# mcveanlab/Corticall

Measured on AMD Instinct MI355X. Metric: k-mers traversed/sec (whole node) + contigs/sec, k=47 3-color LdBG, higher is better.
Workload: dtype u64

## Files before the change

### corticall_amd/csrc/walk.cpp

```cpp
#include <algorithm>
#include <chrono>
#include <numeric>
#include <thread>

#include "lscoop.h"
#include "runs.h"
#include "runstep.h"
#include "shard.h"
#include "strand.h"

namespace ldbg {

#define LDBG_STREAM_BLOCK 64
#define LDBG_STREAM_GRID 65536

LDBG_DEV void walk_finish(const WalkArgs& a, StrandState& st) {
    strand_finish(a, st);
    const bool good = !st.branch_null && st.status == ST_OK;
    a.strand_n[st.s] = good ? st.gV : 0u;
    a.strand_c[st.s] = good ? st.pw.n : 0u;
}

template <int W>
LDBG_DEV bool strand_step(const WalkArgs& a, StrandState& st, LinkStoreDev& ls, const StepPre& pre, RunState& rs) {
// ... 474 lines not shown
}
template <int W>
LDBG_KERNEL void k_contigs(ContigArgs a) {
    const int k = a.g.k;
    const int64_t wave = global_tid() >> 6, lane = global_tid() & 63, nwaves = (global_nthreads() + 63) >> 6;
    for (int64_t i = wave; i < a.n; i += nwaves) {
        if (a.walk_len[i] == 0) continue;
        const int64_t L = a.contig_off[i + 1] - a.contig_off[i];
        const int64_t ro = a.strand_off[2 * i], nr = a.strand_off[2 * i + 1] - ro;
        const int64_t fo = a.strand_off[2 * i + 1];
        const int64_t nrev = nr > 0 ? nr - 1 : 0;
        char* o = a.out + a.contig_off[i];
        if (a.quirk[2 * i] | a.quirk[2 * i + 1]) {
            for (int64_t p = lane; p < L; p += 64) {
                const int64_t v = p < k ? 0 : p - k + 1;
                const Kmer<W> km = walk_vertex_kmer<W>(a, i, v, ro, nr, fo);
                o[p] = "ACGT"[kmer_base<W>(km, k, p < k ? (int)p : k - 1)];
            }
            continue;
        }
        Kmer<W> sk;
#pragma unroll
        for (int w = 0; w < W; w++) sk.w[w] = a.seeds[i * W + w];
        for (int64_t p = lane; p < L; p += 64) {
            unsigned b;
            if (p < nrev) b = path_base(a.dense[ro + (nr - 1 - p)]);
            else if (p < nrev + k) b = kmer_base<W>(sk, k, (int)(p - nrev));
            else b = path_base(a.dense[fo + (p - nrev - k + 1)]);
            o[p] = "ACGT"[b];
        }
    }
}

struct ContigRleArgs {
    GraphView g;
    RunIndexView runs;
    int64_t n;
    const uint64_t* seeds;
    const uint64_t* pool; const uint32_t* block_table; int max_blocks;
    const uint32_t* strand_c; const uint32_t* strand_n;
    const int64_t* walk_len; const int64_t* contig_off;
    char* out;
};
LDBG_DEV uint64_t rle_stored(const ContigRleArgs& a, int64_t s, uint32_t j) {
    return a.pool[(uint64_t)a.block_table[s * a.max_blocks + j / LDBG_PATH_BLOCK] * LDBG_PATH_BLOCK + (j & (LDBG_PATH_BLOCK - 1))];
}
template <int W>
LDBG_KERNEL void k_contigs_rle(ContigRleArgs a) {
    const int k = a.g.k;
    const int64_t wave = global_tid() / wave_size(), nwaves = (global_nthreads() + wave_size() - 1) / wave_size();
    const uint32_t lane = (uint32_t)wave_lane(), WS = (uint32_t)wave_size();
    for (int64_t i = wave; i < a.n; i += nwaves) {
        if (a.walk_len[i] == 0) continue;
        char* o = a.out + a.contig_off[i];
        const int64_t nr = a.strand_n[2 * i], nrev = nr > 0 ? nr - 1 : 0;
        Kmer<W> sk;
#pragma unroll
        for (int w = 0; w < W; w++) sk.w[w] = a.seeds[i * W + w];
        for (uint32_t p = lane; p < (uint32_t)k; p += WS) o[nrev + p] = "ACGT"[kmer_base<W>(sk, k, (int)p)];
        for (int dir = 0; dir < 2; dir++) {
            const int64_t s = 2 * i + dir;
            const bool fwd = dir == 1;
            const uint32_t nc = a.strand_c[s];
            auto place = [&](uint32_t v) -> int64_t { return fwd ? nrev + k - 1 + (int64_t)v : nrev - (int64_t)v; };
            uint32_t base_v = 0;
            uint64_t carry = 0;
            for (uint32_t j0 = 0; j0 < nc; j0 += WS) {
                const uint32_t j = j0 + lane;
                const uint64_t* blk = a.pool + (uint64_t)a.block_table[s * a.max_blocks + j0 / LDBG_PATH_BLOCK] * LDBG_PATH_BLOCK;
                const uint64_t e = j < nc ? LDBG_GLOBAL(const uint64_t, blk)[j & (LDBG_PATH_BLOCK - 1)] : 0ull;
                const uint64_t up = wave_shfl_u64(e, (int)lane - 1);
                const uint64_t prev = (j & (LDBG_PATH_BLOCK - 1)) == 0u ? 0ull : (lane == 0u ? carry : up);
                carry = wave_shfl_u64(e, (int)WS - 1);
                const uint32_t cnt = j < nc ? pd_expanded(prev, e) : 0u;
                const uint32_t incl = wave_incl_scan_u32(cnt);
                const uint32_t at = base_v + incl - cnt;
                const bool head = cnt > 0u && pd_is_head(e);
                if (cnt == 1u && !head && at >= 1u) o[place(at)] = "ACGT"[path_base(e)];
                const bool is_run = head && LDBG_PD_KIND(e) == LDBG_PD_RUN;
                unsigned long long hb = wave_ballot(is_run);
                const uint32_t GS = WS == 64u ? 16u : WS, g = lane / GS, sub = lane % GS;
                const uint8_t* ub = LDBG_GLOBAL(const uint8_t, a.runs.ubase);
                while (hb) {
                    uint32_t myL = 0;
                    bool gv = false;
                    for (uint32_t q = 0; q < WS / GS; q++) {
                        if (!hb) break;
                        const int L = __builtin_ctzll(hb);
                        hb &= hb - 1;
                        if (g == q) { myL = (uint32_t)L; gv = true; }
                    }
                    const uint64_t he = wave_shfl_u64(e, (int)myL);
                    const uint32_t hat = wave_shfl_u32(at, (int)myL), len_of = wave_shfl_u32(cnt, (int)myL);
                    const uint32_t len = gv ? len_of : 0u;
                    const uint64_t next_e = wave_shfl_u64(e, (int)myL + 1);
                    const uint64_t payload = !gv ? 0ull : (myL + 1u < WS ? next_e : rle_stored(a, s, j0 + myL + 1u));
                    const bool asc = (he >> 36) & 1ull, inv = (he >> 37) & 1ull;
                    const uint32_t first = (uint32_t)payload;
                    const unsigned shift = (fwd != inv) ? 2u : 0u, comp = inv ? 3u : 0u;
                    auto ascii = [&](unsigned bb) -> unsigned { return (0x54474341u >> (8u * (((bb >> shift) & 3u) ^ comp))) & 0xFFu; };
                    auto ascii4 = [&](uint32_t bb4) -> uint32_t {
                        const uint32_t f = ((bb4 >> shift) & 0x03030303u) ^ (comp * 0x01010101u);
#ifndef LDBG_HOSTSIM
                        return __builtin_amdgcn_perm(0u, 0x54474341u, f);
#else
                        uint32_t v = 0;
                        for (int bI = 0; bI < 4; bI++) v |= ((0x54474341u >> (8u * ((f >> (8 * bI)) & 3u))) & 0xFFu) << (8 * bI);
                        return v;
#endif
                    };
                    const uint8_t* in_lo = asc ? ub + first : ub + first - (len ? len - 1u : 0u);
                    char* out_lo = LDBG_GLOBAL(char, o) + (fwd ? place(hat) : place(hat + (len ? len - 1u : 0u)));
                    const bool same = asc == fwd;
                    const uint32_t nd = len / 8u;
                    uint32_t max_nd = wave_bcast_u32(nd, 0);
                    for (uint32_t q = 1; q < WS / GS; q++) { const uint32_t o2 = wave_bcast_u32(nd, (int)(q * GS)); max_nd = o2 > max_nd ? o2 : max_nd; }
                    for (uint32_t base = 0; base < max_nd; base += 4u * GS) {
                        uint64_t w[4];
#pragma unroll
                        for (int q = 0; q < 4; q++) {
                            const uint32_t ci = base + (uint32_t)q * GS + sub;
                            w[q] = 0;
                            if (ci < nd) __builtin_memcpy(&w[q], in_lo + (same ? 8u * ci : len - 8u - 8u * ci), 8);
                        }
#pragma unroll
                        for (int q = 0; q < 4; q++) {
                            const uint32_t ci = base + (uint32_t)q * GS + sub;
                            uint64_t v = (uint64_t)ascii4((uint32_t)w[q]) | ((uint64_t)ascii4((uint32_t)(w[q] >> 32)) << 32);
                            if (!same) v = __builtin_bswap64(v);
                            if (ci < nd) __builtin_memcpy(out_lo + 8u * ci, &v, 8);
                        }
                    }
                    for (uint32_t t = 8u * nd + sub; t < len; t += GS) {
                        const unsigned bb = in_lo[same ? t : len - 1u - t];
                        out_lo[t] = (char)ascii(bb);
                    }
                }
                hb = wave_ballot(head && !is_run);
                while (hb) {
                    const int L = __builtin_ctzll(hb);
                    hb &= hb - 1;
                    const uint32_t hat = wave_bcast_u32(at, L), len = wave_bcast_u32(cnt, L);
                    const uint64_t payload = (uint32_t)L + 1u < WS ? wave_bcast_u64(e, L + 1) : rle_stored(a, s, j0 + (uint32_t)L + 1);
                    wave_fence();
                    const uint32_t first = (uint32_t)payload, period = (uint32_t)(payload >> 32);
                    const uint32_t nch = (len + 7u) / 8u;
                    for (uint32_t c = lane; c < nch; c += WS) {
                        const uint32_t t0 = 8u * c, m = len - t0 < 8u ? len - t0 : 8u;
                        uint32_t r = t0 % period;
                        uint64_t v = 0;
#pragma unroll
                        for (uint32_t b = 0; b < 8u; b++) {
                            if (b < m) {
                                const uint64_t ch = (uint8_t)LDBG_GLOBAL(const char, o)[place(first + period + r)];
                                v |= ch << (8u * (fwd ? b : m - 1u - b));
                            }
                            r++;
                            if (r == period) r = 0;
                        }
                        char* lo = LDBG_GLOBAL(char, o) + (fwd ? place(hat + t0) : place(hat + t0 + m - 1u));
                        if (m == 8u) __builtin_memcpy(lo, &v, 8);
                        else for (uint32_t b = 0; b < m; b++) lo[b] = (char)(v >> (8u * b));
                    }
                }
                base_v += wave_bcast_u32(incl, (int)WS - 1);
            }
        }
    }
}

template <int W>
LDBG_KERNEL void k_walk_vertices(GraphView g, const uint64_t* dense, int64_t ro, int64_t nr, int64_t fo, int64_t nf,
                                 const uint64_t* term_r, const uint64_t* term_f, int64_t len, uint64_t* words, int64_t* rec,
                                 int32_t* copy, int32_t* index) {
    const int64_t nrev = nr > 0 ? nr - 1 : 0;
    for (int64_t p = global_tid(); p < len; p += global_nthreads()) {
        uint64_t e;
        int idx_label;
        const uint64_t* term;
        if (p < nrev) { e = dense[ro + (nr - 1 - p)]; idx_label = -1; term = term_r; }
        else if (p == nrev) { e = nr > 0 ? dense[ro] : dense[fo]; idx_label = 0; term = nullptr; }
        else { e = dense[fo + (p - nrev)]; idx_label = 1; term = term_f; }
        int64_t ri = path_idx(e);
        Kmer<W> km;
        if (ri >= 0) {
            km = graph_key<W>(g, ri);
            if (path_flip(e)) km = kmer_revcomp<W>(km, g.k);
        } else {
            for (int w = 0; w < W; w++) km.w[w] = term ? term[w] : 0;
        }
        for (int w = 0; w < W; w++) words[p * W + w] = km.w[w];
        rec[p] = ri;
        copy[p] = path_copy(e);
        index[p] = idx_label;
    }
}

struct RoiHitArgs {
    const uint32_t* roi_of;
    int64_t n;
    const uint64_t* dense; const int64_t* strand_off; const int64_t* walk_len;
// ... 630 lines not shown
        if (!us.empty())
            fprintf(stderr, "[ldbg] %zu strands of %u iterations: us/iter p0/p10/p50/p90/p100 = %.2f %.2f %.2f %.2f %.2f\n", us.size(), max_it,
                    us[0], us[us.size() / 10], us[us.size() / 2], us[us.size() * 9 / 10], us.back());
    }
    double tot_ms = 0; for (int64_t i = 0; i < ns; i++) tot_ms += (tt[2 * i + 1] - tt[2 * i]) / 1e5;
    fprintf(stderr, "[ldbg] sum of strand durations %.1f s over %lld strands; %llu wavefront loop iterations in %d wavefronts\n", tot_ms / 1e3, (long long)ns,
            ctr[14], grid);
    rt::dfree(a.st_times);
}

bool Engine::walk_finish(WalkRun& r, int64_t* traversed) {
    rt::stream_t s = stream_;
    const WalkArgs& a = r.a;
    WalkChunk& out = r.out;
    const int64_t n = r.n, ns = r.ns;
    HostLaps laps;

    if (!h_small_) h_small_ = (unsigned long long*)rt::hmalloc_pinned(64 * 8);
    unsigned long long* const ctr = h_small_;
    if (runs_ && !a.img_on) {
        r.d_retry = (uint32_t*)rt::tmalloc((size_t)ns * 4);
        LDBG_LAUNCH(k_retry_list, grid_for(ns, 256, 1024), 256, s, (const uint32_t*)r.d_status, ns, r.d_retry, r.d_ctr + 28);
        rt::d2h(ctr, r.d_ctr, 256, s);
        rt::stream_sync(s);
        if (r.timed) { r.walk_ms += rt::Event::elapsed_ms(r.ev0, r.ev1); r.timed = false; }
        const int64_t n_again = (int64_t)ctr[28];
        if (n_again > 0) {
            rt::dmemset(r.d_ctr, 0, 8, s);
            WalkArgs b = a;
            b.e.runs = RunIndexView{nullptr, nullptr, nullptr};
            b.retry = r.d_retry;
            b.n_strands = n_again;
            retried_strands_ += n_again;
            launch_k_walk(r, b, s);
        }
    }

    int64_t* d_walk_len = (int64_t*)rt::tmalloc((size_t)n * 8);
    uint8_t* d_seed_ok = (uint8_t*)rt::tmalloc((size_t)n);
    uint32_t* d_contig_len = (uint32_t*)rt::tmalloc((size_t)n * 4);
    int64_t* d_strand_off = (int64_t*)rt::tmalloc((size_t)(ns + 1) * 8);
    int64_t* d_contig_off = (int64_t*)rt::tmalloc((size_t)(n + 1) * 8);
    unsigned long long* d_scan = (unsigned long long*)rt::tmalloc((size_t)(2 * OFF_SCAN_OWNERS + 2) * 8);
    auto free_results = [&] {
        rt::tfree(d_walk_len); rt::tfree(d_seed_ok); rt::tfree(d_contig_len); rt::tfree(d_strand_off); rt::tfree(d_contig_off); rt::tfree(d_scan);
        d_walk_len = nullptr; d_seed_ok = nullptr; d_contig_len = nullptr; d_strand_off = nullptr; d_contig_off = nullptr; d_scan = nullptr;
    };
    AsmArgs aa;
    aa.e = view; aa.n = n; aa.op_and = cfg.combination_operator == LDBG_OP_AND; aa.k = r.k;
    aa.seeds = a.seeds; aa.pool = a.pool; aa.block_table = a.block_table; aa.max_blocks = r.max_blocks;
    aa.strand_n = r.d_strand_n; aa.status = r.d_status; aa.iters = r.d_iters; aa.quirk = r.d_quirk;
    aa.walk_len = d_walk_len; aa.seed_ok = d_seed_ok; aa.contig_len = d_contig_len; aa.flags = r.d_ctr + 24;
    LDBG_LAUNCH(k_walk_lengths, grid_for(n, 256, 2048), 256, s, aa);
    int64_t* d_totals = (int64_t*)(d_scan + 2 * OFF_SCAN_OWNERS);
    launch_offsets(r.d_strand_n, ns, d_strand_off, d_scan, d_totals, s);
    launch_offsets(d_contig_len, n, d_contig_off, d_scan + OFF_SCAN_OWNERS, d_totals + 1, s);
    rt::d2h(ctr, r.d_ctr, 256, s);
    rt::d2h(ctr + 32, d_totals, 16, s);
    rt::stream_sync(s);
    if (r.timed) { r.walk_ms += rt::Event::elapsed_ms(r.ev0, r.ev1); r.timed = false; }
    {
        static const char* const kind_names[8] = {"walk_steps_run", "walk_run_vertices", "walk_steps_lean", "walk_steps_general", "walk_link_adds", "walk_choices",
                                                  "walk_wave_iterations", "walk_wave_general"};
        for (int q = 0; q < 8; q++) profile_add(kind_names[q], (double)ctr[8 + q]);
        profile_add("walk_busiest_general", (double)(ctr[16] >> 32));
        profile_add("walk_busiest_iterations", (double)(ctr[16] & 0xFFFFFFFFull));
// ... 14 lines not shown

    if (pool_full) {
        r.discard(); free_results();
        return false;
    }
    if (any_error) {
        for (int64_t i = 0; i < ns; i++) {
            const uint32_t st = out.status[i];
            if (st != ST_NULLPTR && st != ST_LINKSTORE_FULL && st != ST_COPY_OVERFLOW) continue;
            r.discard(); free_results();
            if (st == ST_NULLPTR)
                throw StatusError(LDBG_ERR_NULLPOINTER, "getNextVertices: record missing while recruitment colours are set (seed " + std::to_string(r.first + i / 2) + ")");
            if (st == ST_LINKSTORE_FULL) throw StatusError(LDBG_ERR_CAPACITY, "LINKSTORE_FULL");
            throw StatusError(LDBG_ERR_UNSUPPORTED, "a vertex was visited more than 32767 times in one walk");
        }
    }
    *traversed += (int64_t)ctr[27];
    out.total_entries = (int64_t)ctr[32];
    out.total_bytes = (int64_t)ctr[33];
    out.host_ready = false;

    const bool lazy = !any_quirk && r.first == 0 && n == batch_n && !getenv("LDBG_EAGER_PATHS");
    out.d_contigs = result_alloc((size_t)out.total_bytes, &out.contigs_cap);
    out.d_strand_off = d_strand_off; d_strand_off = nullptr;
    out.d_contig_off = d_contig_off;
    out.d_walk_len = d_walk_len;
    out.d_strand_c = r.d_strand_c; r.d_strand_c = nullptr;
    out.max_blocks = r.max_blocks;
    out.runs = a.e.runs;
    out.dense_pending = true;
    laps.lap("result buffers");
    rt::Event c0, c1;
    c0.record(s);
    if (lazy) {
        ContigRleArgs ra;
        ra.g = graph->view; ra.runs = a.e.runs; ra.n = n; ra.seeds = a.seeds;
        ra.pool = (const uint64_t*)d_pool_; ra.block_table = (const uint32_t*)d_block_table_; ra.max_blocks = r.max_blocks;
        ra.strand_c = (const uint32_t*)out.d_strand_c; ra.strand_n = r.d_strand_n; ra.walk_len = d_walk_len; ra.contig_off = d_contig_off;
        ra.out = (char*)out.d_contigs;
        int rb = LDBG_STREAM_BLOCK, rcap = LDBG_STREAM_GRID;
#ifndef LDBG_HOSTSIM
        if (const char* ev = getenv("LDBG_RLE_BLOCK")) rb = atoi(ev) >= 256 ? 256 : (atoi(ev) >= 128 ? 128 : 64);
        if (const char* ev = getenv("LDBG_RLE_GRID")) rcap = std::max(1, atoi(ev));
#endif
        LDBG_LAUNCH_W(r.W, k_contigs_rle, grid_for(n * 64, rb, rcap), rb, s, ra);
    } else {
        ensure_dense(out);
        ContigArgs ca;
        ca.g = graph->view; ca.n = n; ca.seeds = a.seeds; ca.dense = (const uint64_t*)out.d_path; ca.strand_off = (const int64_t*)out.d_strand_off;
        ca.walk_len = d_walk_len; ca.contig_off = d_contig_off; ca.quirk = r.d_quirk; ca.term = (const uint64_t*)out.d_term;
        ca.out = (char*)out.d_contigs;
        LDBG_LAUNCH_W(r.W, k_contigs, grid_for(n * 64), 256, s, ca);
    }
    c1.record(s);
    rt::stream_sync(s);
    profile_add("contig", rt::Event::elapsed_ms(c0, c1));
    laps.lap("paths + contigs");
    r.free_tmp();
    d_walk_len = nullptr; d_contig_off = nullptr;
    free_results();
    laps.lap("frees");
    return true;
}


void Engine::sharded_walk_begin(ShardImage& img, const char* seeds, int64_t n, const int32_t* d_seed_slot, rt::stream_t round_stream) {
    if (cfg.stopping_rule != LDBG_STOP_CONTIG || cfg.connect_all_neighbors || cfg.n_secondary > 0)
        throw StatusError(LDBG_ERR_UNSUPPORTED, "walks over a sharded table run ContigStopper without connectAllNeighbors / secondary colours");
    if (&img.graph() != graph) throw StatusError(LDBG_ERR_ARG, "the engine was not created on this image's graph");
    enter();
    sharded_abort();
    clear_batch();
    seeds_to_device(seeds, n, false);
    batch_n = n;
    sharded_run_ = new WalkRun;
    sharded_img_ = &img;
    sharded_stream_ = round_stream ? round_stream : stream_;
    try {
        walk_prepare(0, n, *sharded_run_, &img, d_seed_slot);
        rt::stream_sync(stream_);
    } catch (...) { sharded_abort(); throw; }
}
void Engine::sharded_abort() {
    if (sharded_run_) {
        quiesce();
        sharded_run_->discard();
        delete sharded_run_;
        sharded_run_ = nullptr;
    }
    sharded_img_ = nullptr;
}
// ... 138 lines not shown
```

Before: 187.3 billion.

## Restructure RLE contig emission into a per-wave run table with a flattened chunk copy

The RLE contig kernel now preloads the first two wave-groups of path entries for both strands and hoists the per-contig metadata loads. It builds a shared-memory table of run descriptors and then copies all run chunks in one flat, software-pipelined pass across lanes, instead of handling runs four at a time in 16-lane groups. The goal is to remove lane imbalance and serialized per-run loops in contig materialization. In exchange it adds shared-memory use, binary searches over the table, extra fences, a fallback path for long strands, and the block size is now fixed at 64 threads per block.

```diff
diff --git a/corticall_amd/csrc/walk.cpp b/corticall_amd/csrc/walk.cpp
--- a/corticall_amd/csrc/walk.cpp
+++ b/corticall_amd/csrc/walk.cpp
@@ -540,131 +540,260 @@
     const int64_t* walk_len; const int64_t* contig_off;
     char* out;
 };
-LDBG_DEV uint64_t rle_stored(const ContigRleArgs& a, int64_t s, uint32_t j) {
-    return a.pool[(uint64_t)a.block_table[s * a.max_blocks + j / LDBG_PATH_BLOCK] * LDBG_PATH_BLOCK + (j & (LDBG_PATH_BLOCK - 1))];
+struct alignas(16) RleRun {
+    uint32_t c0;
+    uint32_t in_lo;
+    uint32_t out_lo;
+    uint32_t lenf;
+};
+#define LDBG_RLE_TABLE 64u
+#define LDBG_RLE_HELD 2
+LDBG_DEV uint32_t ascii4(uint32_t bb4, unsigned shift, unsigned comp) {
+    const uint32_t f = ((bb4 >> shift) & 0x03030303u) ^ (comp * 0x01010101u);
+#ifndef LDBG_HOSTSIM
+    return __builtin_amdgcn_perm(0u, 0x54474341u, f);
+#else
+    uint32_t v = 0;
+    for (int bI = 0; bI < 4; bI++) v |= ((0x54474341u >> (8u * ((f >> (8 * bI)) & 3u))) & 0xFFu) << (8 * bI);
+    return v;
+#endif
 }
 template <int W>
-LDBG_KERNEL void k_contigs_rle(ContigRleArgs a) {
-    const int k = a.g.k;
+LDBG_DEV void contigs_rle_wave(const int k, const int64_t n, const int max_blocks, const uint64_t* __restrict__ seeds, const uint64_t* __restrict__ pool,
+                               const uint32_t* __restrict__ block_table, const uint32_t* __restrict__ strand_c, const uint32_t* __restrict__ strand_n,
+                               const int64_t* __restrict__ walk_len, const int64_t* __restrict__ contig_off, const uint8_t* __restrict__ ubase,
+                               char* __restrict__ out, RleRun* tab) {
     const int64_t wave = global_tid() / wave_size(), nwaves = (global_nthreads() + wave_size() - 1) / wave_size();
     const uint32_t lane = (uint32_t)wave_lane(), WS = (uint32_t)wave_size();
-    for (int64_t i = wave; i < a.n; i += nwaves) {
-        if (a.walk_len[i] == 0) continue;
-        char* o = a.out + a.contig_off[i];
-        const int64_t nr = a.strand_n[2 * i], nrev = nr > 0 ? nr - 1 : 0;
+    const uint8_t* ub = LDBG_GLOBAL(const uint8_t, ubase);
+    for (int64_t i = wave; i < n; i += nwaves) {
+        const int64_t wl = walk_len[i], co = contig_off[i];
+        const uint32_t nr = strand_n[2 * i], nc0 = strand_c[2 * i], nc1 = strand_c[2 * i + 1];
+        const uint32_t bt0 = block_table[(2 * i) * max_blocks], bt1 = block_table[(2 * i + 1) * max_blocks];
         Kmer<W> sk;
 #pragma unroll
-        for (int w = 0; w < W; w++) sk.w[w] = a.seeds[i * W + w];
+        for (int w = 0; w < W; w++) sk.w[w] = seeds[i * W + w];
+        if (wl == 0) continue;
+        char* o = out + co;
+        const uint32_t nrev = nr > 0u ? nr - 1u : 0u;
+        auto place = [&](bool fwd, uint32_t v) -> uint32_t { return fwd ? nrev + (uint32_t)k - 1u + v : nrev - v; };
+        uint64_t e[2][LDBG_RLE_HELD], ex[2];
+#pragma unroll
+        for (int d = 0; d < 2; d++) {
+            const uint32_t nc = d ? nc1 : nc0;
+            const uint64_t* blk = pool + (uint64_t)(d ? bt1 : bt0) * LDBG_PATH_BLOCK;
+#pragma unroll
+            for (int g = 0; g < LDBG_RLE_HELD; g++) {
+                const uint32_t j = (uint32_t)g * WS + lane;
+                e[d][g] = j < nc ? LDBG_GLOBAL(const uint64_t, blk)[j] : 0ull;
+            }
+            ex[d] = LDBG_RLE_HELD * WS < nc ? LDBG_GLOBAL(const uint64_t, blk)[LDBG_RLE_HELD * WS] : 0ull;
+        }
         for (uint32_t p = lane; p < (uint32_t)k; p += WS) o[nrev + p] = "ACGT"[kmer_base<W>(sk, k, (int)p)];
-        for (int dir = 0; dir < 2; dir++) {
-            const int64_t s = 2 * i + dir;
-            const bool fwd = dir == 1;
-            const uint32_t nc = a.strand_c[s];
-            auto place = [&](uint32_t v) -> int64_t { return fwd ? nrev + k - 1 + (int64_t)v : nrev - (int64_t)v; };
-            uint32_t base_v = 0;
-            uint64_t carry = 0;
-            for (uint32_t j0 = 0; j0 < nc; j0 += WS) {
+
+        struct Group { uint32_t at, cnt; bool is_run, is_rep; uint64_t payload; };
+        auto scan_group = [&](bool fwd, uint32_t j0, uint32_t nc, uint64_t ge, uint64_t after, uint64_t& carry, uint32_t& base_v) -> Group {
+            Group r;
+            const uint32_t j = j0 + lane;
+            const uint64_t up = wave_shfl_u64(ge, (int)lane - 1), dn = wave_shfl_u64(ge, (int)lane + 1);
+            const uint64_t prev = (j & (LDBG_PATH_BLOCK - 1)) == 0u ? 0ull : (lane == 0u ? carry : up);
+            carry = wave_shfl_u64(ge, (int)WS - 1);
+            r.payload = lane + 1u < WS ? dn : after;
+            r.cnt = j < nc ? pd_expanded(prev, ge) : 0u;
+            const uint32_t incl = wave_incl_scan_u32(r.cnt);
+            r.at = base_v + incl - r.cnt;
+            const bool head = r.cnt > 0u && pd_is_head(ge);
+            if (r.cnt == 1u && !head && r.at >= 1u) o[place(fwd, r.at)] = "ACGT"[path_base(ge)];
+            r.is_run = head && LDBG_PD_KIND(ge) == LDBG_PD_RUN;
+            r.is_rep = head && !r.is_run;
+            base_v += wave_bcast_u32(incl, (int)WS - 1);
+            return r;
+        };
+        auto table_add = [&](bool fwd, uint64_t ge, const Group& gr, uint32_t& R, uint32_t& C) {
+            const unsigned long long hb = wave_ballot(gr.is_run);
+            const uint32_t len = gr.is_run ? gr.cnt : 0u, nch = (len + 7u) / 8u;
+            const uint32_t incl = wave_incl_scan_u32(nch);
+            if (gr.is_run) {
+                const bool asc = (ge >> 36) & 1ull, inv = (ge >> 37) & 1ull;
+                const uint32_t first = (uint32_t)gr.payload, span = len ? len - 1u : 0u;
+                RleRun t;
+                t.c0 = C + incl - nch;
+                t.in_lo = asc ? first : first - span;
+                t.out_lo = fwd ? place(fwd, gr.at) : place(fwd, gr.at + span);
+                t.lenf = len | ((asc == fwd) ? 1u << 20 : 0u) | ((fwd != inv) ? 1u << 21 : 0u) | (inv ? 1u << 22 : 0u);
+                tab[R + (uint32_t)wave_count_below(hb)] = t;
+            }
+            R += (uint32_t)__builtin_popcountll(hb);
+            C += wave_bcast_u32(incl, (int)WS - 1);
+        };
+        auto copy_pass = [&](const uint32_t R, const uint32_t C) {
+            if (R == 0u || C == 0u) return;
+            uint32_t r = 0, nxt = 0;
+            RleRun cur = tab[0];
+            auto load1 = [&](uint32_t c, uint64_t& w, uint32_t& oo, uint32_t& mf) {
+                w = 0; oo = 0; mf = 0;
+                if (c >= C) return;
+                if (c >= nxt) {
+                    uint32_t lo = r, hi = R;
+                    while (hi - lo > 1u) { const uint32_t mid = (lo + hi) >> 1; if (tab[mid].c0 <= c) lo = mid; else hi = mid; }
+                    r = lo; cur = tab[r]; nxt = r + 1u < R ? tab[r + 1u].c0 : 0xFFFFFFFFu;
+                }
+                const uint32_t len = cur.lenf & 0xFFFFFu, t0 = 8u * (c - cur.c0), m = len - t0 < 8u ? len - t0 : 8u;
+                const bool same = (cur.lenf >> 20) & 1u;
+                oo = cur.out_lo + t0; mf = m | ((cur.lenf >> 20) << 4);
+                const uint8_t* in = ub + cur.in_lo;
+                if (len >= 8u) {
+                    const uint32_t x = same ? (t0 < len - 8u ? t0 : len - 8u) : (len - 8u > t0 ? len - 8u - t0 : 0u);
+                    __builtin_memcpy(&w, in + x, 8);
+                } else {
+#pragma unroll
+                    for (uint32_t b = 0; b < 7u; b++)
+                        if (b < len) w |= (uint64_t)in[b] << (8u * (same ? b + 8u - len : b));
+                }
+            };
+            auto store1 = [&](uint64_t w, uint32_t oo, uint32_t mf) {
+                const uint32_t m = mf & 15u;
+                if (!m) return;
+                const unsigned shift = (mf >> 5) & 1u ? 2u : 0u, comp = (mf >> 6) & 1u ? 3u : 0u;
+                uint64_t v = (uint64_t)ascii4((uint32_t)w, shift, comp) | ((uint64_t)ascii4((uint32_t)(w >> 32), shift, comp) << 32);
+                if (!((mf >> 4) & 1u)) v = __builtin_bswap64(v);
+                v >>= 8u * (8u - m);
+                char* p = LDBG_GLOBAL(char, o) + oo;
+                if (m == 8u) __builtin_memcpy(p, &v, 8);
+                else {
+#pragma unroll
+                    for (uint32_t b = 0; b < 7u; b++)
+                        if (b < m) p[b] = (char)(v >> (8u * b));
+                }
+            };
+            const uint32_t NB = (C + 4u * WS - 1u) / (4u * WS);
+            uint64_t wa[4], wb[4];
+            uint32_t oa[4], ob[4], ma[4], mb[4];
+#pragma unroll
+            for (uint32_t q = 0; q < 4u; q++) load1(q * WS + lane, wa[q], oa[q], ma[q]);
+            for (uint32_t b = 0; b < NB; b++) {
+#pragma unroll
+                for (uint32_t q = 0; q < 4u; q++) load1((4u * (b + 1u) + q) * WS + lane, wb[q], ob[q], mb[q]);
+#pragma unroll
+                for (uint32_t q = 0; q < 4u; q++) store1(wa[q], oa[q], ma[q]);
+#pragma unroll
+                for (uint32_t q = 0; q < 4u; q++) { wa[q] = wb[q]; oa[q] = ob[q]; ma[q] = mb[q]; }
+            }
+        };
+        auto repeat_tail = [&](bool fwd, uint32_t hat, uint32_t len, uint64_t payload) {
+            wave_fence();
+            const uint32_t first = (uint32_t)payload, period = (uint32_t)(payload >> 32);
+            const uint32_t nch = (len + 7u) / 8u;
+            for (uint32_t c = lane; c < nch; c += WS) {
+                const uint32_t t0 = 8u * c, m = len - t0 < 8u ? len - t0 : 8u;
+                uint32_t r = t0 % period;
+                uint64_t v = 0;
+#pragma unroll
+                for (uint32_t b = 0; b < 8u; b++) {
+                    if (b < m) {
+                        const uint64_t ch = (uint8_t)LDBG_GLOBAL(const char, o)[place(fwd, first + period + r)];
+                        v |= ch << (8u * (fwd ? b : m - 1u - b));
+                    }
+                    r++;
+                    if (r == period) r = 0;
+                }
+                char* lo = LDBG_GLOBAL(char, o) + (fwd ? place(fwd, hat + t0) : place(fwd, hat + t0 + m - 1u));
+                if (m == 8u) __builtin_memcpy(lo, &v, 8);
+                else for (uint32_t b = 0; b < m; b++) lo[b] = (char)(v >> (8u * b));
+            }
+        };
+        auto repeat_of = [&](bool fwd, const Group& gr) {
+            const unsigned long long hb = wave_ballot(gr.is_rep);
+            if (!hb) return;
+            const int L = __builtin_ctzll(hb);
+            repeat_tail(fwd, wave_bcast_u32(gr.at, L), wave_bcast_u32(gr.cnt, L), wave_bcast_u64(gr.payload, L));
+        };
+
+        Group gr[2][LDBG_RLE_HELD];
+        uint64_t carry[2] = {0ull, 0ull};
+        uint32_t base_v[2] = {0u, 0u}, heads = 0;
+#pragma unroll
+        for (int d = 0; d < 2; d++) {
+            const uint32_t nc = d ? nc1 : nc0;
+#pragma unroll
+            for (int g = 0; g < LDBG_RLE_HELD; g++) {
+                const uint64_t after = g + 1 < LDBG_RLE_HELD ? wave_bcast_u64(e[d][g + 1 < LDBG_RLE_HELD ? g + 1 : g], 0) : ex[d];
+                gr[d][g] = scan_group(d == 1, (uint32_t)g * WS, nc, e[d][g], after, carry[d], base_v[d]);
+                heads += (uint32_t)__builtin_popcountll(wave_ballot(gr[d][g].is_run));
+            }
+        }
+        const bool joint = heads <= LDBG_RLE_TABLE;
+#pragma nounroll
+        for (int pass = 0; pass < (joint ? 1 : 2); pass++) {
+            uint32_t R = 0, C = 0;
+#pragma unroll
+            for (int d = 0; d < 2; d++) {
+                if (!joint && d != pass) continue;
+#pragma unroll
+                for (int g = 0; g < LDBG_RLE_HELD; g++) table_add(d == 1, e[d][g], gr[d][g], R, C);
+            }
+            wave_fence();
+            copy_pass(R, C);
+            wave_fence();
+        }
+#pragma nounroll
+        for (int d = 0; d < 2; d++) {
+            Group last = gr[0][0];
+#pragma unroll
+            for (int g = 0; g < LDBG_RLE_HELD; g++) {
+                const Group& x = d ? gr[1][g] : gr[0][g];
+                if (g == 0) last = x;
+                else { const bool any = wave_ballot(x.is_rep) != 0ull; if (any) last = x; }
+            }
+            repeat_of(d == 1, last);
+        }
+
+#pragma nounroll
+        for (int d = 0; d < 2; d++) {
+            const uint32_t nc = d ? nc1 : nc0;
+            if (nc <= LDBG_RLE_HELD * WS) continue;
+            const bool fwd = d == 1;
+            const uint32_t* btp = block_table + (2 * i + d) * max_blocks;
+            uint32_t bcur = d ? bt1 : bt0, bnext = nc > LDBG_PATH_BLOCK ? btp[1] : 0u;
+            uint64_t cy = d ? carry[1] : carry[0];
+            uint32_t bv = d ? base_v[1] : base_v[0];
+            auto entries = [&](uint32_t j0) -> uint64_t {
                 const uint32_t j = j0 + lane;
-                const uint64_t* blk = a.pool + (uint64_t)a.block_table[s * a.max_blocks + j0 / LDBG_PATH_BLOCK] * LDBG_PATH_BLOCK;
-                const uint64_t e = j < nc ? LDBG_GLOBAL(const uint64_t, blk)[j & (LDBG_PATH_BLOCK - 1)] : 0ull;
-                const uint64_t up = wave_shfl_u64(e, (int)lane - 1);
-                const uint64_t prev = (j & (LDBG_PATH_BLOCK - 1)) == 0u ? 0ull : (lane == 0u ? carry : up);
-                carry = wave_shfl_u64(e, (int)WS - 1);
-                const uint32_t cnt = j < nc ? pd_expanded(prev, e) : 0u;
-                const uint32_t incl = wave_incl_scan_u32(cnt);
-                const uint32_t at = base_v + incl - cnt;
-                const bool head = cnt > 0u && pd_is_head(e);
-                if (cnt == 1u && !head && at >= 1u) o[place(at)] = "ACGT"[path_base(e)];
-                const bool is_run = head && LDBG_PD_KIND(e) == LDBG_PD_RUN;
-                unsigned long long hb = wave_ballot(is_run);
-                const uint32_t GS = WS == 64u ? 16u : WS, g = lane / GS, sub = lane % GS;
-                const uint8_t* ub = LDBG_GLOBAL(const uint8_t, a.runs.ubase);
-                while (hb) {
-                    uint32_t myL = 0;
-                    bool gv = false;
-                    for (uint32_t q = 0; q < WS / GS; q++) {
-                        if (!hb) break;
-                        const int L = __builtin_ctzll(hb);
-                        hb &= hb - 1;
-                        if (g == q) { myL = (uint32_t)L; gv = true; }
+                return j < nc ? LDBG_GLOBAL(const uint64_t, pool + (uint64_t)bcur * LDBG_PATH_BLOCK)[j & (LDBG_PATH_BLOCK - 1)] : 0ull;
+            };
+            uint64_t ec = entries(LDBG_RLE_HELD * WS);
+            for (uint32_t j0 = LDBG_RLE_HELD * WS; j0 < nc; j0 += WS) {
+                const uint32_t jn = j0 + WS;
+                uint64_t en = 0;
+                if (jn < nc) {
+                    if ((jn & (LDBG_PATH_BLOCK - 1)) == 0u) {
+                        const uint32_t bi = jn / LDBG_PATH_BLOCK + 1u;
+                        bcur = bnext;
+                        bnext = (uint64_t)bi * LDBG_PATH_BLOCK < nc ? btp[bi] : 0u;
                     }
-                    const uint64_t he = wave_shfl_u64(e, (int)myL);
-                    const uint32_t hat = wave_shfl_u32(at, (int)myL), len_of = wave_shfl_u32(cnt, (int)myL);
-                    const uint32_t len = gv ? len_of : 0u;
-                    const uint64_t next_e = wave_shfl_u64(e, (int)myL + 1);
-                    const uint64_t payload = !gv ? 0ull : (myL + 1u < WS ? next_e : rle_stored(a, s, j0 + myL + 1u));
-                    const bool asc = (he >> 36) & 1ull, inv = (he >> 37) & 1ull;
-                    const uint32_t first = (uint32_t)payload;
-                    const unsigned shift = (fwd != inv) ? 2u : 0u, comp = inv ? 3u : 0u;
-                    auto ascii = [&](unsigned bb) -> unsigned { return (0x54474341u >> (8u * (((bb >> shift) & 3u) ^ comp))) & 0xFFu; };
-                    auto ascii4 = [&](uint32_t bb4) -> uint32_t {
-                        const uint32_t f = ((bb4 >> shift) & 0x03030303u) ^ (comp * 0x01010101u);
+                    en = entries(jn);
+                }
+                const Group x = scan_group(fwd, j0, nc, ec, wave_bcast_u64(en, 0), cy, bv);
+                uint32_t R = 0, C = 0;
+                table_add(fwd, ec, x, R, C);
+                wave_fence();
+                copy_pass(R, C);
+                wave_fence();
+                repeat_of(fwd, x);
+                ec = en;
+            }
+        }
+    }
+}
+template <int W>
+LDBG_WAVE_KERNEL void k_contigs_rle(ContigRleArgs a) {
 #ifndef LDBG_HOSTSIM
-                        return __builtin_amdgcn_perm(0u, 0x54474341u, f);
+    __shared__ RleRun tab[LDBG_RLE_TABLE];
 #else
-                        uint32_t v = 0;
-                        for (int bI = 0; bI < 4; bI++) v |= ((0x54474341u >> (8u * ((f >> (8 * bI)) & 3u))) & 0xFFu) << (8 * bI);
-                        return v;
-#endif
-                    };
-                    const uint8_t* in_lo = asc ? ub + first : ub + first - (len ? len - 1u : 0u);
-                    char* out_lo = LDBG_GLOBAL(char, o) + (fwd ? place(hat) : place(hat + (len ? len - 1u : 0u)));
-                    const bool same = asc == fwd;
-                    const uint32_t nd = len / 8u;
-                    uint32_t max_nd = wave_bcast_u32(nd, 0);
-                    for (uint32_t q = 1; q < WS / GS; q++) { const uint32_t o2 = wave_bcast_u32(nd, (int)(q * GS)); max_nd = o2 > max_nd ? o2 : max_nd; }
-                    for (uint32_t base = 0; base < max_nd; base += 4u * GS) {
-                        uint64_t w[4];
-#pragma unroll
-                        for (int q = 0; q < 4; q++) {
-                            const uint32_t ci = base + (uint32_t)q * GS + sub;
-                            w[q] = 0;
-                            if (ci < nd) __builtin_memcpy(&w[q], in_lo + (same ? 8u * ci : len - 8u - 8u * ci), 8);
-                        }
-#pragma unroll
-                        for (int q = 0; q < 4; q++) {
-                            const uint32_t ci = base + (uint32_t)q * GS + sub;
-                            uint64_t v = (uint64_t)ascii4((uint32_t)w[q]) | ((uint64_t)ascii4((uint32_t)(w[q] >> 32)) << 32);
-                            if (!same) v = __builtin_bswap64(v);
-                            if (ci < nd) __builtin_memcpy(out_lo + 8u * ci, &v, 8);
-                        }
-                    }
-                    for (uint32_t t = 8u * nd + sub; t < len; t += GS) {
-                        const unsigned bb = in_lo[same ? t : len - 1u - t];
-                        out_lo[t] = (char)ascii(bb);
-                    }
-                }
-                hb = wave_ballot(head && !is_run);
-                while (hb) {
-                    const int L = __builtin_ctzll(hb);
-                    hb &= hb - 1;
-                    const uint32_t hat = wave_bcast_u32(at, L), len = wave_bcast_u32(cnt, L);
-                    const uint64_t payload = (uint32_t)L + 1u < WS ? wave_bcast_u64(e, L + 1) : rle_stored(a, s, j0 + (uint32_t)L + 1);
-                    wave_fence();
-                    const uint32_t first = (uint32_t)payload, period = (uint32_t)(payload >> 32);
-                    const uint32_t nch = (len + 7u) / 8u;
-                    for (uint32_t c = lane; c < nch; c += WS) {
-                        const uint32_t t0 = 8u * c, m = len - t0 < 8u ? len - t0 : 8u;
-                        uint32_t r = t0 % period;
-                        uint64_t v = 0;
-#pragma unroll
-                        for (uint32_t b = 0; b < 8u; b++) {
-                            if (b < m) {
-                                const uint64_t ch = (uint8_t)LDBG_GLOBAL(const char, o)[place(first + period + r)];
-                                v |= ch << (8u * (fwd ? b : m - 1u - b));
-                            }
-                            r++;
-                            if (r == period) r = 0;
-                        }
-                        char* lo = LDBG_GLOBAL(char, o) + (fwd ? place(hat + t0) : place(hat + t0 + m - 1u));
-                        if (m == 8u) __builtin_memcpy(lo, &v, 8);
-                        else for (uint32_t b = 0; b < m; b++) lo[b] = (char)(v >> (8u * b));
-                    }
-                }
-                base_v += wave_bcast_u32(incl, (int)WS - 1);
-            }
-        }
-    }
+    static thread_local RleRun tab[LDBG_RLE_TABLE];
+#endif
+    contigs_rle_wave<W>(a.g.k, a.n, a.max_blocks, a.seeds, a.pool, a.block_table, a.strand_c, a.strand_n, a.walk_len, a.contig_off,
+                        a.runs.ubase, a.out, tab);
 }
 
 template <int W>
@@ -1447,12 +1576,11 @@
         ra.pool = (const uint64_t*)d_pool_; ra.block_table = (const uint32_t*)d_block_table_; ra.max_blocks = r.max_blocks;
         ra.strand_c = (const uint32_t*)out.d_strand_c; ra.strand_n = r.d_strand_n; ra.walk_len = d_walk_len; ra.contig_off = d_contig_off;
         ra.out = (char*)out.d_contigs;
-        int rb = LDBG_STREAM_BLOCK, rcap = LDBG_STREAM_GRID;
+        int rcap = LDBG_STREAM_GRID;
 #ifndef LDBG_HOSTSIM
-        if (const char* ev = getenv("LDBG_RLE_BLOCK")) rb = atoi(ev) >= 256 ? 256 : (atoi(ev) >= 128 ? 128 : 64);
         if (const char* ev = getenv("LDBG_RLE_GRID")) rcap = std::max(1, atoi(ev));
 #endif
-        LDBG_LAUNCH_W(r.W, k_contigs_rle, grid_for(n * 64, rb, rcap), rb, s, ra);
+        LDBG_LAUNCH_W(r.W, k_contigs_rle, grid_for(n * 64, LDBG_STREAM_BLOCK, rcap), LDBG_STREAM_BLOCK, s, ra);
     } else {
         ensure_dense(out);
         ContigArgs ca;
```

After: 190.0 billion, median of 6. +1.4%, better.

## Split RLE contig emission into per-strand scan, work-queue copy, and repeat kernels

Applied to the files above, without the earlier changes.

The per-contig RLE kernel now assigns one wave per strand instead of per contig. Instead of copying run payloads inline, it emits fixed-size copy work items (runs cut into pieces) and repeat items into global queues through atomic counters. Separate kernels then drain those queues: a grouped copy kernel for runs and a wave-per-item kernel for periodic repeats. This is meant to remove the load imbalance from long runs serialised within one wave. The cost is extra launches, temporary buffers sized from counters, and atomics, and the repeat kernel relies on earlier output being complete before it runs.

```diff
diff --git a/corticall_amd/csrc/walk.cpp b/corticall_amd/csrc/walk.cpp
--- a/corticall_amd/csrc/walk.cpp
+++ b/corticall_amd/csrc/walk.cpp
@@ -530,6 +530,16 @@
     }
 }
 
+#define LDBG_CONTIG_CUT 2048u
+#define LDBG_COPY_GROUP 16
+#define LDBG_COPY_GRID 16384
+#define LDBG_REPEAT_GRID 256
+struct RepeatItem { uint32_t strand, hat, len, first, period, pad; };
+#ifdef LDBG_HOSTSIM
+struct ContigDebug { uint64_t v[9] = {0, 0, 0, 0, 0, 0, 0, 0, 0}; };
+inline ContigDebug& contig_debug() { static ContigDebug d; return d; }
+extern "C" void ldbg_debug_contigs(uint64_t* out) { for (int q = 0; q < 9; q++) out[q] = contig_debug().v[q]; contig_debug() = ContigDebug(); }
+#endif
 struct ContigRleArgs {
     GraphView g;
     RunIndexView runs;
@@ -539,6 +549,10 @@
     const uint32_t* strand_c; const uint32_t* strand_n;
     const int64_t* walk_len; const int64_t* contig_off;
     char* out;
+    uint64_t* items;
+    RepeatItem* reps;
+    unsigned long long* counts;
+    uint32_t cut;
 };
 LDBG_DEV uint64_t rle_stored(const ContigRleArgs& a, int64_t s, uint32_t j) {
     return a.pool[(uint64_t)a.block_table[s * a.max_blocks + j / LDBG_PATH_BLOCK] * LDBG_PATH_BLOCK + (j & (LDBG_PATH_BLOCK - 1))];
@@ -548,121 +562,179 @@
     const int k = a.g.k;
     const int64_t wave = global_tid() / wave_size(), nwaves = (global_nthreads() + wave_size() - 1) / wave_size();
     const uint32_t lane = (uint32_t)wave_lane(), WS = (uint32_t)wave_size();
-    for (int64_t i = wave; i < a.n; i += nwaves) {
+    for (int64_t s = wave; s < 2 * a.n; s += nwaves) {
+        const int64_t i = s >> 1;
         if (a.walk_len[i] == 0) continue;
+        const bool fwd = (s & 1) != 0;
+        const int64_t co = a.contig_off[i];
+        char* o = a.out + co;
+        const int64_t nr = a.strand_n[2 * i], nrev = nr > 0 ? nr - 1 : 0;
+        if (fwd) {
+            Kmer<W> sk;
+#pragma unroll
+            for (int w = 0; w < W; w++) sk.w[w] = a.seeds[i * W + w];
+            for (uint32_t p = lane; p < (uint32_t)k; p += WS) o[nrev + p] = "ACGT"[kmer_base<W>(sk, k, (int)p)];
+        }
+        const uint32_t nc = a.strand_c[s];
+#ifdef LDBG_HOSTSIM
+        if (lane == 0u) { ContigDebug& d = contig_debug(); if (nc > d.v[3]) d.v[3] = nc; if (nc > LDBG_PATH_BLOCK) d.v[4]++; }
+#endif
+        auto place = [&](uint32_t v) -> int64_t { return fwd ? nrev + k - 1 + (int64_t)v : nrev - (int64_t)v; };
+        uint32_t base_v = 0;
+        uint64_t carry = 0;
+        for (uint32_t j0 = 0; j0 < nc; j0 += WS) {
+            const uint32_t j = j0 + lane;
+            const uint64_t* blk = a.pool + (uint64_t)a.block_table[s * a.max_blocks + j0 / LDBG_PATH_BLOCK] * LDBG_PATH_BLOCK;
+            const uint64_t e = j < nc ? LDBG_GLOBAL(const uint64_t, blk)[j & (LDBG_PATH_BLOCK - 1)] : 0ull;
+            const uint64_t up = wave_shfl_u64(e, (int)lane - 1);
+            const uint64_t next_e = wave_shfl_u64(e, (int)lane + 1);
+            const uint64_t prev = (j & (LDBG_PATH_BLOCK - 1)) == 0u ? 0ull : (lane == 0u ? carry : up);
+            carry = wave_shfl_u64(e, (int)WS - 1);
+            const uint32_t cnt = j < nc ? pd_expanded(prev, e) : 0u;
+            const uint32_t incl = wave_incl_scan_u32(cnt);
+            const uint32_t at = base_v + incl - cnt;
+            const bool head = cnt > 0u && pd_is_head(e);
+            if (cnt == 1u && !head && at >= 1u) o[place(at)] = "ACGT"[path_base(e)];
+            const bool is_run = head && LDBG_PD_KIND(e) == LDBG_PD_RUN;
+            const uint32_t pieces = is_run ? (cnt + a.cut - 1u) / a.cut : 0u;
+            const uint32_t incl_p = wave_incl_scan_u32(pieces);
+            const uint32_t tot_p = wave_bcast_u32(incl_p, (int)WS - 1);
+            uint64_t slot0 = 0;
+            if (tot_p) {
+                unsigned long long b = 0;
+                if (lane == 0u) b = atomic_add_u64(a.counts, (unsigned long long)tot_p);
+                slot0 = wave_bcast_u64(b, 0);
+            }
+            const uint64_t payload = !head ? 0ull : (lane + 1u < WS ? next_e : rle_stored(a, s, j + 1u));
+            if (is_run) {
+                const uint32_t len = cnt;
+                const bool asc = (e >> 36) & 1ull, inv = (e >> 37) & 1ull;
+                const uint32_t first = (uint32_t)payload;
+#ifdef LDBG_HOSTSIM
+                {
+                    ContigDebug& d = contig_debug();
+                    d.v[0] += pieces; if (pieces > 1u) d.v[1]++;
+                    if (lane + 1u == WS && WS > 1u) d.v[2]++;
+                    d.v[5] |= 1ull << ((fwd ? 4 : 0) + (asc ? 2 : 0) + (inv ? 1 : 0));
+                    if (len > 8u) d.v[6] |= 1ull << (len % 8u); else d.v[7] |= 1ull << len;
+                }
+#endif
+                const uint32_t in_lo = asc ? first : first - (len - 1u);
+                const int64_t out_lo = co + (fwd ? place(at) : place(at + len - 1u));
+                const bool same = asc == fwd;
+                const uint64_t bits = (same ? 1ull << 52 : 0ull) | ((fwd != inv) ? 1ull << 53 : 0ull) | (inv ? 1ull << 54 : 0ull);
+                uint64_t* it = LDBG_GLOBAL(uint64_t, a.items) + 2u * (slot0 + incl_p - pieces);
+                for (uint32_t t = 0; t < len; t += a.cut, it += 2) {
+                    const uint32_t pl = len - t < a.cut ? len - t : a.cut;
+                    it[0] = (uint64_t)(same ? in_lo + t : in_lo + (len - t - pl)) | ((uint64_t)pl << 32) | bits;
+                    it[1] = (uint64_t)(out_lo + (int64_t)t);
+                }
+            }
+            if (head && !is_run) {
+                const unsigned long long slot = atomic_add_u64(a.counts + 1, 1ull);
+#ifdef LDBG_HOSTSIM
+                contig_debug().v[8]++;
+#endif
+                RepeatItem r;
+                r.strand = (uint32_t)s; r.hat = at; r.len = cnt; r.first = (uint32_t)payload; r.period = (uint32_t)(payload >> 32); r.pad = 0u;
+                LDBG_GLOBAL(RepeatItem, a.reps)[slot] = r;
+            }
+            base_v += wave_bcast_u32(incl, (int)WS - 1);
+        }
+    }
+}
+
+LDBG_DEV uint32_t contig_ascii4(uint32_t bb4, unsigned shift, unsigned comp) {
+    const uint32_t f = ((bb4 >> shift) & 0x03030303u) ^ (comp * 0x01010101u);
+#ifndef LDBG_HOSTSIM
+    return __builtin_amdgcn_perm(0u, 0x54474341u, f);
+#else
+    uint32_t v = 0;
+    for (int bI = 0; bI < 4; bI++) v |= ((0x54474341u >> (8u * ((f >> (8 * bI)) & 3u))) & 0xFFu) << (8 * bI);
+    return v;
+#endif
+}
+struct ContigCopyArgs {
+    const uint64_t* items;
+    const unsigned long long* count;
+    const uint8_t* ubase;
+    char* out;
+};
+template <int G>
+LDBG_KERNEL void k_contig_copy(ContigCopyArgs a) {
+    const uint32_t GS = (uint32_t)wave_size() < (uint32_t)G ? (uint32_t)wave_size() : (uint32_t)G;
+    const uint64_t grp = (uint64_t)global_tid() / GS, ngrp = (uint64_t)global_nthreads() / GS;
+    const uint32_t sub = (uint32_t)((uint64_t)global_tid() % GS);
+    const uint64_t n_items = *a.count;
+    if (ngrp == 0) return;
+    for (uint64_t it = grp; it < n_items; it += ngrp) {
+        const uint64_t w0 = a.items[2 * it], dst = a.items[2 * it + 1];
+        const uint32_t len = (uint32_t)(w0 >> 32) & 0xFFFFFu;
+        const bool same = (w0 >> 52) & 1ull;
+        const unsigned shift = ((w0 >> 53) & 1ull) ? 2u : 0u, comp = ((w0 >> 54) & 1ull) ? 3u : 0u;
+        const uint8_t* in_lo = LDBG_GLOBAL(const uint8_t, a.ubase) + (uint32_t)w0;
+        char* out_lo = LDBG_GLOBAL(char, a.out) + dst;
+        const uint32_t nd = len / 8u;
+        for (uint32_t base = 0; base < nd; base += 4u * GS) {
+            uint64_t w[4];
+#pragma unroll
+            for (int q = 0; q < 4; q++) {
+                const uint32_t ci = base + (uint32_t)q * GS + sub;
+                w[q] = 0;
+                if (ci < nd) __builtin_memcpy(&w[q], in_lo + (same ? 8u * ci : len - 8u - 8u * ci), 8);
+            }
+#pragma unroll
+            for (int q = 0; q < 4; q++) {
+                const uint32_t ci = base + (uint32_t)q * GS + sub;
+                uint64_t v = (uint64_t)contig_ascii4((uint32_t)w[q], shift, comp) | ((uint64_t)contig_ascii4((uint32_t)(w[q] >> 32), shift, comp) << 32);
+                if (!same) v = __builtin_bswap64(v);
+                if (ci < nd) __builtin_memcpy(out_lo + 8u * ci, &v, 8);
+            }
+        }
+        for (uint32_t t = 8u * nd + sub; t < len; t += GS) {
+            const unsigned bb = in_lo[same ? t : len - 1u - t];
+            out_lo[t] = (char)((0x54474341u >> (8u * (((bb >> shift) & 3u) ^ comp))) & 0xFFu);
+        }
+    }
+}
+
+struct ContigRepeatArgs {
+    const RepeatItem* reps;
+    const unsigned long long* count;
+    int k;
+    const uint32_t* strand_n; const int64_t* contig_off;
+    char* out;
+};
+LDBG_KERNEL void k_contig_repeats(ContigRepeatArgs a) {
+    const int64_t wave = global_tid() / wave_size(), nwaves = (global_nthreads() + wave_size() - 1) / wave_size();
+    const uint32_t lane = (uint32_t)wave_lane(), WS = (uint32_t)wave_size();
+    const int64_t n_items = (int64_t)*a.count;
+    for (int64_t it = wave; it < n_items; it += nwaves) {
+        const RepeatItem r = a.reps[it];
+        const int64_t i = (int64_t)(r.strand >> 1);
+        const bool fwd = (r.strand & 1u) != 0u;
+        const int k = a.k;
+        const int64_t nr = a.strand_n[2 * i], nrev = nr > 0 ? nr - 1 : 0;
         char* o = a.out + a.contig_off[i];
-        const int64_t nr = a.strand_n[2 * i], nrev = nr > 0 ? nr - 1 : 0;
-        Kmer<W> sk;
+        auto place = [&](uint32_t v) -> int64_t { return fwd ? nrev + k - 1 + (int64_t)v : nrev - (int64_t)v; };
+        const uint32_t hat = r.hat, len = r.len, first = r.first, period = r.period;
+        const uint32_t nch = (len + 7u) / 8u;
+        for (uint32_t c = lane; c < nch; c += WS) {
+            const uint32_t t0 = 8u * c, m = len - t0 < 8u ? len - t0 : 8u;
+            uint32_t rr = t0 % period;
+            uint64_t v = 0;
 #pragma unroll
-        for (int w = 0; w < W; w++) sk.w[w] = a.seeds[i * W + w];
-        for (uint32_t p = lane; p < (uint32_t)k; p += WS) o[nrev + p] = "ACGT"[kmer_base<W>(sk, k, (int)p)];
-        for (int dir = 0; dir < 2; dir++) {
-            const int64_t s = 2 * i + dir;
-            const bool fwd = dir == 1;
-            const uint32_t nc = a.strand_c[s];
-            auto place = [&](uint32_t v) -> int64_t { return fwd ? nrev + k - 1 + (int64_t)v : nrev - (int64_t)v; };
-            uint32_t base_v = 0;
-            uint64_t carry = 0;
-            for (uint32_t j0 = 0; j0 < nc; j0 += WS) {
-                const uint32_t j = j0 + lane;
-                const uint64_t* blk = a.pool + (uint64_t)a.block_table[s * a.max_blocks + j0 / LDBG_PATH_BLOCK] * LDBG_PATH_BLOCK;
-                const uint64_t e = j < nc ? LDBG_GLOBAL(const uint64_t, blk)[j & (LDBG_PATH_BLOCK - 1)] : 0ull;
-                const uint64_t up = wave_shfl_u64(e, (int)lane - 1);
-                const uint64_t prev = (j & (LDBG_PATH_BLOCK - 1)) == 0u ? 0ull : (lane == 0u ? carry : up);
-                carry = wave_shfl_u64(e, (int)WS - 1);
-                const uint32_t cnt = j < nc ? pd_expanded(prev, e) : 0u;
-                const uint32_t incl = wave_incl_scan_u32(cnt);
-                const uint32_t at = base_v + incl - cnt;
-                const bool head = cnt > 0u && pd_is_head(e);
-                if (cnt == 1u && !head && at >= 1u) o[place(at)] = "ACGT"[path_base(e)];
-                const bool is_run = head && LDBG_PD_KIND(e) == LDBG_PD_RUN;
-                unsigned long long hb = wave_ballot(is_run);
-                const uint32_t GS = WS == 64u ? 16u : WS, g = lane / GS, sub = lane % GS;
-                const uint8_t* ub = LDBG_GLOBAL(const uint8_t, a.runs.ubase);
-                while (hb) {
-                    uint32_t myL = 0;
-                    bool gv = false;
-                    for (uint32_t q = 0; q < WS / GS; q++) {
-                        if (!hb) break;
-                        const int L = __builtin_ctzll(hb);
-                        hb &= hb - 1;
-                        if (g == q) { myL = (uint32_t)L; gv = true; }
-                    }
-                    const uint64_t he = wave_shfl_u64(e, (int)myL);
-                    const uint32_t hat = wave_shfl_u32(at, (int)myL), len_of = wave_shfl_u32(cnt, (int)myL);
-                    const uint32_t len = gv ? len_of : 0u;
-                    const uint64_t next_e = wave_shfl_u64(e, (int)myL + 1);
-                    const uint64_t payload = !gv ? 0ull : (myL + 1u < WS ? next_e : rle_stored(a, s, j0 + myL + 1u));
-                    const bool asc = (he >> 36) & 1ull, inv = (he >> 37) & 1ull;
-                    const uint32_t first = (uint32_t)payload;
-                    const unsigned shift = (fwd != inv) ? 2u : 0u, comp = inv ? 3u : 0u;
-                    auto ascii = [&](unsigned bb) -> unsigned { return (0x54474341u >> (8u * (((bb >> shift) & 3u) ^ comp))) & 0xFFu; };
-                    auto ascii4 = [&](uint32_t bb4) -> uint32_t {
-                        const uint32_t f = ((bb4 >> shift) & 0x03030303u) ^ (comp * 0x01010101u);
-#ifndef LDBG_HOSTSIM
-                        return __builtin_amdgcn_perm(0u, 0x54474341u, f);
-#else
-                        uint32_t v = 0;
-                        for (int bI = 0; bI < 4; bI++) v |= ((0x54474341u >> (8u * ((f >> (8 * bI)) & 3u))) & 0xFFu) << (8 * bI);
-                        return v;
-#endif
-                    };
-                    const uint8_t* in_lo = asc ? ub + first : ub + first - (len ? len - 1u : 0u);
-                    char* out_lo = LDBG_GLOBAL(char, o) + (fwd ? place(hat) : place(hat + (len ? len - 1u : 0u)));
-                    const bool same = asc == fwd;
-                    const uint32_t nd = len / 8u;
-                    uint32_t max_nd = wave_bcast_u32(nd, 0);
-                    for (uint32_t q = 1; q < WS / GS; q++) { const uint32_t o2 = wave_bcast_u32(nd, (int)(q * GS)); max_nd = o2 > max_nd ? o2 : max_nd; }
-                    for (uint32_t base = 0; base < max_nd; base += 4u * GS) {
-                        uint64_t w[4];
-#pragma unroll
-                        for (int q = 0; q < 4; q++) {
-                            const uint32_t ci = base + (uint32_t)q * GS + sub;
-                            w[q] = 0;
-                            if (ci < nd) __builtin_memcpy(&w[q], in_lo + (same ? 8u * ci : len - 8u - 8u * ci), 8);
-                        }
-#pragma unroll
-                        for (int q = 0; q < 4; q++) {
-                            const uint32_t ci = base + (uint32_t)q * GS + sub;
-                            uint64_t v = (uint64_t)ascii4((uint32_t)w[q]) | ((uint64_t)ascii4((uint32_t)(w[q] >> 32)) << 32);
-                            if (!same) v = __builtin_bswap64(v);
-                            if (ci < nd) __builtin_memcpy(out_lo + 8u * ci, &v, 8);
-                        }
-                    }
-                    for (uint32_t t = 8u * nd + sub; t < len; t += GS) {
-                        const unsigned bb = in_lo[same ? t : len - 1u - t];
-                        out_lo[t] = (char)ascii(bb);
-                    }
+            for (uint32_t b = 0; b < 8u; b++) {
+                if (b < m) {
+                    const uint64_t ch = (uint8_t)LDBG_GLOBAL(const char, o)[place(first + period + rr)];
+                    v |= ch << (8u * (fwd ? b : m - 1u - b));
                 }
-                hb = wave_ballot(head && !is_run);
-                while (hb) {
-                    const int L = __builtin_ctzll(hb);
-                    hb &= hb - 1;
-                    const uint32_t hat = wave_bcast_u32(at, L), len = wave_bcast_u32(cnt, L);
-                    const uint64_t payload = (uint32_t)L + 1u < WS ? wave_bcast_u64(e, L + 1) : rle_stored(a, s, j0 + (uint32_t)L + 1);
-                    wave_fence();
-                    const uint32_t first = (uint32_t)payload, period = (uint32_t)(payload >> 32);
-                    const uint32_t nch = (len + 7u) / 8u;
-                    for (uint32_t c = lane; c < nch; c += WS) {
-                        const uint32_t t0 = 8u * c, m = len - t0 < 8u ? len - t0 : 8u;
-                        uint32_t r = t0 % period;
-                        uint64_t v = 0;
-#pragma unroll
-                        for (uint32_t b = 0; b < 8u; b++) {
-                            if (b < m) {
-                                const uint64_t ch = (uint8_t)LDBG_GLOBAL(const char, o)[place(first + period + r)];
-                                v |= ch << (8u * (fwd ? b : m - 1u - b));
-                            }
-                            r++;
-                            if (r == period) r = 0;
-                        }
-                        char* lo = LDBG_GLOBAL(char, o) + (fwd ? place(hat + t0) : place(hat + t0 + m - 1u));
-                        if (m == 8u) __builtin_memcpy(lo, &v, 8);
-                        else for (uint32_t b = 0; b < m; b++) lo[b] = (char)(v >> (8u * b));
-                    }
-                }
-                base_v += wave_bcast_u32(incl, (int)WS - 1);
+                rr++;
+                if (rr == period) rr = 0;
             }
+            char* lo = LDBG_GLOBAL(char, o) + (fwd ? place(hat + t0) : place(hat + t0 + m - 1u));
+            if (m == 8u) __builtin_memcpy(lo, &v, 8);
+            else for (uint32_t b = 0; b < m; b++) lo[b] = (char)(v >> (8u * b));
         }
     }
 }
@@ -1361,6 +1433,7 @@
             b.retry = r.d_retry;
             b.n_strands = n_again;
             retried_strands_ += n_again;
+            profile_add("walk_retried_strands", (double)n_again);
             launch_k_walk(r, b, s);
         }
     }
@@ -1441,18 +1514,38 @@
     laps.lap("result buffers");
     rt::Event c0, c1;
     c0.record(s);
+    uint64_t* d_items = nullptr;
+    void* d_reps = nullptr;
     if (lazy) {
         ContigRleArgs ra;
         ra.g = graph->view; ra.runs = a.e.runs; ra.n = n; ra.seeds = a.seeds;
         ra.pool = (const uint64_t*)d_pool_; ra.block_table = (const uint32_t*)d_block_table_; ra.max_blocks = r.max_blocks;
         ra.strand_c = (const uint32_t*)out.d_strand_c; ra.strand_n = r.d_strand_n; ra.walk_len = d_walk_len; ra.contig_off = d_contig_off;
         ra.out = (char*)out.d_contigs;
-        int rb = LDBG_STREAM_BLOCK, rcap = LDBG_STREAM_GRID;
+        ra.cut = LDBG_CONTIG_CUT;
+        if (const char* ev = getenv("LDBG_CONTIG_CUT")) ra.cut = (uint32_t)std::max(1, std::min(atoi(ev), 0xFFFFF));
+        const uint64_t heads = std::min<uint64_t>(ctr[8], ctr[1] * (uint64_t)(LDBG_PATH_BLOCK / 2));
+        const uint64_t item_cap = heads + (uint64_t)out.total_bytes / ra.cut;
+        d_items = (uint64_t*)rt::tmalloc((size_t)std::max<uint64_t>(1, item_cap) * 16);
+        d_reps = rt::tmalloc((size_t)ns * sizeof(RepeatItem));
+        ra.items = d_items; ra.reps = (RepeatItem*)d_reps; ra.counts = r.d_ctr + 29;
+        int rb = LDBG_STREAM_BLOCK, rcap = LDBG_STREAM_GRID, cgrid = LDBG_COPY_GRID, cgroup = LDBG_COPY_GROUP;
 #ifndef LDBG_HOSTSIM
         if (const char* ev = getenv("LDBG_RLE_BLOCK")) rb = atoi(ev) >= 256 ? 256 : (atoi(ev) >= 128 ? 128 : 64);
         if (const char* ev = getenv("LDBG_RLE_GRID")) rcap = std::max(1, atoi(ev));
-#endif
-        LDBG_LAUNCH_W(r.W, k_contigs_rle, grid_for(n * 64, rb, rcap), rb, s, ra);
+        if (const char* ev = getenv("LDBG_COPY_GRID")) cgrid = std::max(1, atoi(ev));
+        if (const char* ev = getenv("LDBG_COPY_GROUP")) cgroup = atoi(ev) == 8 ? 8 : 16;
+#endif
+        LDBG_LAUNCH_W(r.W, k_contigs_rle, grid_for(ns * 64, rb, 2 * rcap), rb, s, ra);
+        ContigCopyArgs cc;
+        cc.items = d_items; cc.count = r.d_ctr + 29; cc.ubase = a.e.runs.ubase; cc.out = (char*)out.d_contigs;
+        const int copy_blocks = grid_for((int64_t)std::max<uint64_t>(1, item_cap) * cgroup, 256, cgrid);
+        if (cgroup == 8) LDBG_LAUNCH(k_contig_copy<8>, copy_blocks, 256, s, cc);
+        else LDBG_LAUNCH(k_contig_copy<16>, copy_blocks, 256, s, cc);
+        ContigRepeatArgs cr;
+        cr.reps = (const RepeatItem*)d_reps; cr.count = r.d_ctr + 30; cr.k = r.k; cr.strand_n = r.d_strand_n; cr.contig_off = d_contig_off;
+        cr.out = (char*)out.d_contigs;
+        LDBG_LAUNCH(k_contig_repeats, LDBG_REPEAT_GRID, LDBG_STREAM_BLOCK, s, cr);
     } else {
         ensure_dense(out);
         ContigArgs ca;
@@ -1466,6 +1559,7 @@
     profile_add("contig", rt::Event::elapsed_ms(c0, c1));
     laps.lap("paths + contigs");
     r.free_tmp();
+    rt::tfree(d_items); rt::tfree(d_reps);
     d_walk_len = nullptr; d_contig_off = nullptr;
     free_results();
     laps.lap("frees");
```

Result: slower. 186.3 billion before, 118.9 billion after (-36.2%).
